# vibhaska/delta

Hardware: AMD Instinct MI355X
Metric: log actions replayed/sec + achieved HBM GB/s, 1/2/4/8 GPU, 10M-file table (higher is better)
Workload: dtype u8/int64; 1 GPU; config 3: 10M-file checkpoint + 30 JSON commits, 16000032 actions -> 10000000 live files, 30% remove/re-add churn, retention cutoff; actions=16000032, json_bytes=1775145997, checkpoint_bytes=859787616, parallelism=single GPU

## Files before the change

delta_amd/csrc/engine.hip:

```cpp
#include <hip/hip_runtime.h>
#include <rccl/rccl.h>
#include <dlfcn.h>
#include <sys/mman.h>
#include <unistd.h>
#include <sys/stat.h>
#include <fcntl.h>
#include <thread>

#include <algorithm>
#include <cmath>
#include <atomic>
#include <functional>
#include <type_traits>
#include <cstring>
#include <cctype>
#include <cerrno>
#include <cstdlib>
#include <cstdio>
#include <map>
#include <chrono>
#include <condition_variable>
#include <memory>
#include <mutex>
#include <string>
// ... 484 lines not shown
  std::vector<std::string> paths;
  std::vector<int> max_def, max_rep;
  std::vector<bool> present;
  std::vector<uint64_t> levels;
  std::vector<PageDesc> pages;
  DBuf<PageDesc> d_pages;
  uint32_t dict_entries = 0;
  DBuf<uint8_t> d_arena;
  std::vector<SnapPage> snap_pages;
  std::vector<uint32_t> chunk_base, block_page, chunk_page;
  std::vector<CopyJob> copy_jobs;
  uint32_t nchunks = 0;
  DBuf<SnapPage> d_snap;
  DBuf<uint32_t> d_chunk_base, d_block_page, d_chunk_page;
  DBuf<CopyJob> d_copy;
  DBuf<uint32_t> s_spec_exit, s_vis, s_entry, s_spec_first, s_assumed, s_region, s_chunk_out, s_chunk_out_start,
      s_chunk_elems, s_pages_bad, s_block_chunk, s_page_mark;
  DBuf<uint8_t> s_chunk_flag;
  DBuf<unsigned long long> s_region_count;
  std::vector<uint32_t> wg_chunk0;
  DBuf<uint32_t> d_wg_chunk0;
  uint64_t snap_in_bytes = 0, snap_out_bytes = 0, copy_bytes = 0;
  uint64_t snap_elements = 0;
  std::vector<InflatePage> gz_pages;
  DBuf<InflatePage> d_gz;
  uint64_t gz_in_bytes = 0, gz_out_bytes = 0;
  uint32_t ba_pages = 0;
  uint64_t ba_vals = 0;
  std::vector<uint2> ba_tiles;
  DBuf<uint2> d_ba_tiles;
  DBuf<uint32_t> s_ba_vals, s_ba_ok, s_ba_count, s_ba_tile_cnt;
  DBuf<uint64_t> s_ba_tile_off, s_ba_kept;
  DBuf<uint32_t> s_ba_link;
  std::vector<uint32_t> dl_pages;
  uint32_t dl_fc = 0, dl_groups = 0, dl_chunks = 0;
  uint64_t dl_tab = 0, dl_blk = 0;
  DBuf<uint32_t> d_dl_pages, s_dl_cnt;
  DBuf<uint64_t> s_dl_tab, s_dl_blk, s_dl_size, d_dl_out, d_dl_sized;
  DBuf<uint8_t> dl_arena;
  std::vector<uint64_t> dl_out, dl_sized_bytes;
  bool dl_sized = false;
  uint64_t dl_sizings = 0, dl_arena_bytes = 0;
};

struct HostBytes {
  uint8_t* p = nullptr;
  size_t n = 0, cap = 0;
  bool pinned = false;
  HostBytes() = default;
  HostBytes(const HostBytes&) = delete;
  HostBytes& operator=(const HostBytes&) = delete;
  ~HostBytes() { release(); }
  void release() {
    if (p) {
      if (pinned) (void)hipHostFree(p);
      else std::free(p);
    }
    p = nullptr;
    n = cap = 0;
  }
  void alloc(size_t bytes, size_t pad, bool pin) {
    release();
    cap = bytes + pad;
    pinned = pin;
    if (pin && hipHostMalloc(reinterpret_cast<void**>(&p), std::max<size_t>(cap, 1), hipHostMallocDefault) != hipSuccess) {
      (void)hipGetLastError();
// ... 492 lines not shown
    dbuf = DBuf<T>(s.ctx, vec.size());
    if (!vec.empty())
      HIP_OK(hipMemcpyAsync(dbuf.p, vec.data(), vec.size() * sizeof(T), hipMemcpyHostToDevice, s.ctx->stream));
  };
  up(P.d_snap, P.snap_pages);
  if (!P.gz_pages.empty()) up(P.d_gz, P.gz_pages);
  up(P.d_chunk_base, P.chunk_base);
  up(P.d_chunk_page, P.chunk_page);
  up(P.d_block_page, P.block_page);
  up(P.d_copy, P.copy_jobs);
  up(P.d_wg_chunk0, P.wg_chunk0);
  P.s_spec_exit = DBuf<uint32_t>(s.ctx, P.nchunks);
  P.s_vis = DBuf<uint32_t>(s.ctx, uint64_t(P.nchunks) * (snappy_chunk_bytes() / 32));
  P.s_entry = DBuf<uint32_t>(s.ctx, P.nchunks);
  P.s_spec_first = DBuf<uint32_t>(s.ctx, P.nchunks);
  P.s_assumed = DBuf<uint32_t>(s.ctx, P.nchunks);
  P.s_region = DBuf<uint32_t>(s.ctx, P.nchunks);
  P.s_block_chunk = DBuf<uint32_t>(s.ctx, P.block_page.size() + 1);
  P.s_chunk_flag = DBuf<uint8_t>(s.ctx, P.nchunks);
  P.s_region_count = DBuf<unsigned long long>(s.ctx, 1);
  P.s_chunk_out = DBuf<uint32_t>(s.ctx, P.nchunks);
  P.s_chunk_out_start = DBuf<uint32_t>(s.ctx, P.nchunks);
  P.s_chunk_elems = DBuf<uint32_t>(s.ctx, P.nchunks);
  P.s_pages_bad = DBuf<uint32_t>(s.ctx, P.snap_pages.size());
  P.s_page_mark = DBuf<uint32_t>(s.ctx, P.snap_pages.size());
  P.s_ba_vals = DBuf<uint32_t>(s.ctx, P.ba_vals);
  up(P.d_ba_tiles, P.ba_tiles);
  P.s_ba_tile_cnt = DBuf<uint32_t>(s.ctx, P.ba_tiles.size());
  P.s_ba_tile_off = DBuf<uint64_t>(s.ctx, P.ba_tiles.size() + 1);
  P.s_ba_kept = DBuf<uint64_t>(s.ctx, P.ba_tiles.size() * 256);
  P.s_ba_link = DBuf<uint32_t>(s.ctx, P.ba_tiles.size() * 3);
  P.s_ba_ok = DBuf<uint32_t>(s.ctx, P.ba_pages);
  P.s_ba_count = DBuf<uint32_t>(s.ctx, P.ba_pages);
  if (!P.dl_pages.empty()) {
    std::stable_partition(P.dl_pages.begin(), P.dl_pages.end(), [&](uint32_t i) { return P.pages[i].encoding == 7; });
    for (size_t k = 0; k < P.dl_pages.size(); ++k) {
      PageDesc& d = P.pages[P.dl_pages[k]];
      d.dl_slot = uint32_t(k);
      if (d.encoding == 7) {
        ++P.dl_fc;
        P.dl_groups = std::max(P.dl_groups, (d.num_values + 63) / 64);
      }
    }
    up(P.d_dl_pages, P.dl_pages);
    P.s_dl_tab = DBuf<uint64_t>(s.ctx, P.dl_tab);
    P.s_dl_blk = DBuf<uint64_t>(s.ctx, 2 * P.dl_blk);
    P.s_dl_cnt = DBuf<uint32_t>(s.ctx, P.dl_pages.size());
    P.s_dl_size = DBuf<uint64_t>(s.ctx, 2 * P.dl_pages.size());
    P.d_dl_out = DBuf<uint64_t>(s.ctx, P.dl_pages.size());
    P.d_dl_sized = DBuf<uint64_t>(s.ctx, P.dl_pages.size());
  }
  for (PageDesc& d : P.pages) {
    d.src = pqb + d.src;
    d.dst = arb + d.dst;
  }
  up(P.d_pages, P.pages);
}

static uint64_t scan_scratch_for(uint64_t n) {
  uint64_t b = scan_scratch_bytes(std::max<uint64_t>(n, uint64_t(1) << 23));
  if (const char* cap = std::getenv("DR_SCAN_SCRATCH_MAX")) b = std::min<uint64_t>(b, std::strtoull(cap, nullptr, 10));
  return b;
}
static ScanScratch ss(const DBuf<uint8_t>& b) { return ScanScratch{b.p, b.n}; }

static void pq_error(const PagePlan& P, uint32_t code, uint32_t gz, const std::string& what) {
// ... 1 lines not shown
    const uint32_t k = ~gz;
    const char* col = k < P.gz_pages.size() ? P.paths[size_t(P.pages[P.gz_pages[k].page].col)].c_str() : "?";
    fail(DR_E_PARQUET, fmt("corrupt gzip page in %s", col));
  }
  if (code != 0) fail(DR_E_PARQUET, fmt("%s failed (code %u)", what.c_str(), code));
}
static void pq_error(const PagePlan& P, const DBuf<uint32_t>& err, hipStream_t stream, const std::string& what) {
  const std::vector<uint32_t> w = d2h(err.p, 2, stream);
  pq_error(P, w[0], w[1], what);
}

static void decode_pages(dr_ctx* ctx, PagePlan& P, ParquetArgs& pa, DBuf<uint64_t>& dict_ptr, DBuf<uint32_t>& dict_len,
                         DBuf<uint32_t>& err, void*) {
  hipStream_t stream = ctx->stream;
  DBuf<uint8_t> own_scratch(ctx, scan_scratch_for(std::max<uint64_t>(P.nchunks, P.ba_tiles.size())));
  const ScanScratch scratch = ss(own_scratch);
  pa.pages = P.d_pages.p;
  pa.npages = uint32_t(P.pages.size());
  dict_ptr = DBuf<uint64_t>(ctx, P.dict_entries);
  dict_len = DBuf<uint32_t>(ctx, P.dict_entries);
  pa.dict_ptr = dict_ptr.p;
  pa.dict_len = dict_len.p;
  pa.error = err.p;
  pa.ba_vals = P.s_ba_vals.p;
  pa.ba_hit = nullptr;
  pa.ba_tiles = P.d_ba_tiles.p;
  pa.nba_tiles = uint32_t(P.ba_tiles.size());
  pa.ba_tile_cnt = P.s_ba_tile_cnt.p;
  pa.ba_tile_off = P.s_ba_tile_off.p;
  pa.ba_kept = P.s_ba_kept.p;
  pa.ba_link = P.s_ba_link.p;
  pa.ba_ok = P.s_ba_ok.p;
  pa.ba_count = P.s_ba_count.p;
  launch_page_copy(P.d_copy.p, uint32_t(P.copy_jobs.size()), stream);
  if (!P.snap_pages.empty()) {
    P.s_pages_bad.zero(stream);
    P.s_page_mark.zero(stream);
    P.s_chunk_flag.zero(stream);
    P.s_region_count.zero(stream);
    SnappyArgs sa{};
    sa.pages = P.d_snap.p;
    sa.npages = uint32_t(P.snap_pages.size());
    sa.chunk_base = P.d_chunk_base.p;
    sa.nchunks = P.nchunks;
    sa.spec_exit = P.s_spec_exit.p;
    sa.vis = P.s_vis.p;
    sa.entry = P.s_entry.p;
    sa.spec_first = P.s_spec_first.p;
    sa.assumed_exit = P.s_assumed.p;
    sa.chunk_flag = P.s_chunk_flag.p;
    sa.region = P.s_region.p;
    sa.region_count = P.s_region_count.p;
    sa.page_mark = P.s_page_mark.p;
    sa.chunk_out = P.s_chunk_out.p;
    sa.chunk_out_start = P.s_chunk_out_start.p;
    sa.chunk_elems = P.s_chunk_elems.p;
    sa.block_page = P.d_block_page.p;
    sa.block_chunk = P.s_block_chunk.p;
    sa.nblocks = uint32_t(P.block_page.size());
    sa.wg_chunk0 = P.d_wg_chunk0.p;
    sa.nwg = uint32_t(P.wg_chunk0.size());
    sa.pages_bad = P.s_pages_bad.p;
    sa.error = err.p;
    sa.chunk_page = P.d_chunk_page.p;
    DBuf<uint64_t> stamps, rstats;
    const bool dbg = std::getenv("DR_SNAP_DEBUG") != nullptr;
// ... 108 lines not shown
    pa.dl_tab = P.s_dl_tab.p;
    pa.dl_blk = P.s_dl_blk.p;
    pa.dl_cnt = P.s_dl_cnt.p;
    pa.dl_size = P.s_dl_size.p;
    launch_dl_scan(pa, stream);
    if (P.dl_fc) {
      if (!P.dl_sized) {
        const std::vector<uint64_t> sz = d2h(P.s_dl_size.p, 2 * uint64_t(ndl), stream);
        P.dl_out.assign(ndl, 0);
        P.dl_sized_bytes.assign(ndl, 0);
        uint64_t at = 0, longest = 0;
        for (uint32_t k = 0; k < P.dl_fc; ++k) {
          P.dl_out[k] = at;
          P.dl_sized_bytes[k] = sz[2 * k];
          at += (sz[2 * k] + 16 + 15) & ~uint64_t(15);
          longest = std::max(longest, sz[2 * k + 1]);
        }
        P.dl_arena = DBuf<uint8_t>(ctx, at + 64);
        P.dl_arena_bytes = at;
        P.dl_chunks = uint32_t((longest + 63) / 64);
        HIP_OK(hipMemcpyAsync(P.d_dl_out.p, P.dl_out.data(), ndl * sizeof(uint64_t), hipMemcpyHostToDevice, stream));
        HIP_OK(hipMemcpyAsync(P.d_dl_sized.p, P.dl_sized_bytes.data(), ndl * sizeof(uint64_t), hipMemcpyHostToDevice, stream));
        P.dl_sized = true;
        ++P.dl_sizings;
      }
      pa.dl_out = P.d_dl_out.p;
      pa.dl_sized = P.d_dl_sized.p;
      pa.dl_arena = P.dl_arena.p;
      launch_dl_expand(pa, P.dl_fc, P.dl_groups, P.dl_chunks, stream);
    }
  }
  launch_pq_dict(pa, stream);
  launch_pq_data(pa, stream);
}

static double now_s();

static void plan_checkpoint(StagedData& s) {
  const double t0 = now_s();
  uint64_t row_base = 0;
  for (CkPart& part : s.parts) {
    part.meta = pq::parse_footer(s.h_pq.data() + part.off, part.len);
    part.row_base = row_base;
    part.rows = 0;
    for (size_t gi = size_t(part.rg_lo); gi < part.rg_end(); ++gi) part.rows += uint64_t(part.meta.row_groups[gi].num_rows);
    row_base += part.rows;
  }
  s.ck_rows = row_base;
  if (s.parts.empty()) return;
  const pq::FileMeta& m0 = s.parts[0].meta;
  for (int c = 0; c < HC_N; ++c) {
    const pq::Leaf* l = m0.leaf(kHotPath[c]);
    s.has_col[c] = l != nullptr;
    if (l) {
      if (l->max_rep != 0) fail(DR_E_PARQUET, fmt("column %s is repeated", kHotPath[c]));
      s.max_def[c] = l->max_def;
      if (c == HC_ADD_PATH) s.add_def = l->def_of[0];
      if (c == HC_RM_PATH) s.rm_def = l->def_of[0];
    }
  }
  if (!s.has_col[HC_ADD_PATH]) fail(DR_E_PARQUET, "checkpoint has no add.path column");
  s.hot.paths.assign(kHotPath, kHotPath + HC_N);
  const double t1 = now_s();
  plan_pages(s, s.hot);
  const double t2 = now_s();
  for (CkPart& part : s.parts) decode_ck_nonfile(s, part, 0);
  if (std::getenv("DR_STAGE_DEBUG"))
    std::fprintf(stderr, "plan_checkpoint: %zu parts, footers %.3f s, pages %.3f s (%zu pages), non-file rows %.3f s\n",
                 s.parts.size(), t1 - t0, t2 - t1, s.hot.pages.size(), now_s() - t2);
}

struct StageSrc {
  int64_t version = 0;
  int32_t kind = DR_FILE_JSON, part = 0;
  const uint8_t* data = nullptr;
  uint64_t len = 0;
  std::string path;
  int32_t rg_lo = 0, rg_hi = -1;
};

static double now_s() {
  return std::chrono::duration<double>(std::chrono::steady_clock::now().time_since_epoch()).count();
}

static std::shared_ptr<StagedData> stage_sources(dr_ctx* ctx, std::vector<StageSrc>& src) {
  const bool dbg = std::getenv("DR_STAGE_DEBUG") != nullptr;
  const double t0 = now_s();
  auto s = std::make_shared<StagedData>();
  s->ctx = ctx;
  struct FdGuard {
    std::vector<int> fds;
    ~FdGuard() { for (int fd : fds) if (fd >= 0) close(fd); }
  } fdg;
  fdg.fds.assign(src.size(), -1);
  std::vector<uint8_t> ends_nl(src.size(), 0);
// ... 350 lines not shown
        HIP_OK(hipMemset(phase, 0, 16 * sizeof(unsigned long long)));
      }
      ja.phase = phase;
      if (++phase_calls % 200 == 0) {
        unsigned long long h[16];
        HIP_OK(hipMemcpy(h, phase, sizeof(h), hipMemcpyDeviceToHost));
        if (h[4])
          std::fprintf(stderr, "k_json_lines<true> clocks per wave: stage %.0f tape %.0f walk %.0f (rounds %.0f, first round %.0f; tape scan %.0f emit %.0f) (%llu waves)\n",
                       double(h[0]) / double(h[4]), double(h[1]) / double(h[4]), double(h[2]) / double(h[4]),
                       double(h[3]) / double(h[4]), double(h[5]) / double(h[4]), double(h[6]) / double(h[4]),
                       double(h[7]) / double(h[4]), h[4]);
        if (h[8] + h[9] + h[10] + h[11])
          std::fprintf(stderr, "k_apply_commit apply clocks: post-parse %.0f append %.0f touch %.0f delta %.0f\n",
                       double(h[8]) / double(h[4]), double(h[9]) / double(h[4]), double(h[10]) / double(h[4]),
                       double(h[11]) / double(h[4]));
        if (h[12] + h[13])
          std::fprintf(stderr, "k_apply_commit clocks: stage %.0f newlines %.0f walk %.0f apply %.0f expiry %.0f readback %.0f\n",
                       double(h[0]) / double(h[4]), double(h[1]) / double(h[4]), double(h[2]) / double(h[4]),
                       double(h[6]) / double(h[4]), double(h[12]) / double(h[4]), double(h[13]) / double(h[4]));
      }
    }
    if (defer_tail && fuse1 && tail_post) pp.parse_deferred = true;
    else launch_json_parse(ja, s2);
    if (!tail_post) launch_json_hard(ja, s2);
    if (overlap) {
      HIP_OK(hipEventCreateWithFlags(&ov.done, hipEventDisableTiming));
      HIP_OK(hipEventRecord(ov.done, s2));
    }
  }
  DBuf<uint8_t> cdefs;
  DBuf<int64_t> cival[HC_N];
  DBuf<uint64_t> csptr[HC_N];
  DBuf<uint32_t> cslen[HC_N];
  DBuf<uint64_t> dict_ptr;
  DBuf<uint32_t> dict_len, pq_err;
  if (R) {
    DR_STAGE("decode.checkpoint", stream);
    ParquetArgs pa{};
    pa.ncols = HC_N;
    cdefs = DBuf<uint8_t>(ctx, uint64_t(HC_N) * R);
    cdefs.zero(stream);
    for (int c = 0; c < HC_N; ++c) {
      if (c == HC_ADD_PATH || c == HC_RM_PATH) {
        csptr[c] = DBuf<uint64_t>(ctx, R);
        cslen[c] = DBuf<uint32_t>(ctx, R);
      } else {
        cival[c] = DBuf<int64_t>(ctx, R);
      }
      pa.cols[c] = FlatColumn{cdefs.p + uint64_t(c) * R, nullptr, cival[c].p, csptr[c].p, cslen[c].p};
    }
    pq_err = DBuf<uint32_t>(ctx, 2);
    pq_err.zero(stream);
    decode_pages(ctx, s.hot, pa, dict_ptr, dict_len, pq_err, scratch.p);
    CkptAssembleArgs ca{};
    ca.add_path = pa.cols[HC_ADD_PATH];
    ca.add_size = pa.cols[HC_ADD_SIZE];
    ca.rm_path = pa.cols[HC_RM_PATH];
    ca.rm_delts = pa.cols[HC_RM_DELTS];
    ca.add_def = s.add_def;
    ca.rm_def = s.rm_def;
    ca.add_path_max = s.max_def[HC_ADD_PATH];
    ca.add_size_max = s.has_col[HC_ADD_SIZE] ? s.max_def[HC_ADD_SIZE] : 255;
    ca.rm_path_max = s.max_def[HC_RM_PATH];
    ca.rm_delts_max = s.has_col[HC_RM_DELTS] ? s.max_def[HC_RM_DELTS] : 255;
    ca.has_rm = s.has_col[HC_RM_PATH] ? 1 : 0;
    ca.nrows = R;
    ca.row_base = 0;
    ca.act = act;
    ca.special_count = counters.p + 0;
    ca.special_bytes = counters.p + 1;
    launch_ckpt_assemble(ca, stream);
  }
  if (ov.done) {
    HIP_OK(hipStreamWaitEvent(stream, ov.done, 0));
  }
  if (R) HIP_OK(hipMemcpyAsync(counters.p + 7, pq_err.p, 2 * sizeof(uint32_t), hipMemcpyDeviceToDevice, stream));
  if (canonicalize) {
    DR_STAGE("canonicalize", stream);
    int64_t hint = s.canon_need.load();
    if (hint < 0 && ctx->opt.canon_hint >= 0) hint = ctx->opt.canon_hint;
    uint64_t cap = 0;
    if (hint < 0 && R == 0 && json_len <= (uint64_t(64) << 20)) {
// ... 4369 lines not shown
```

delta_amd/csrc/k_parquet.hip:

```cpp
#include "delta_enc.h"
#include "dev_common.h"
#include "kernels.h"

namespace dr {
namespace dev {

enum PqErr : uint32_t { PQE_SNAPPY = 1, PQE_LEVELS = 2, PQE_VALUES = 3, PQE_DICT = 4, PQE_ENCODING = 5 };

__device__ __forceinline__ void set_err(uint32_t* e, uint32_t code) { atomicCAS(e, 0u, code); }

__device__ __forceinline__ int level_width(int max_level) {
  int w = 0;
  while ((1 << w) <= max_level) ++w;
  return max_level == 0 ? 0 : w;
}

struct Rle {
  const uint8_t* p;
  const uint8_t* end;
  int width;
  uint32_t left;
  bool packed;
  uint32_t value;
  const uint8_t* pk;
// ... 212 lines not shown
  const uint64_t nx = p + 4 + w;
  if (nx > S || (w && !(in ? stage_u8(st, k + 4) : b[p + 4]))) return false;
  *next = nx;
  return true;
}
__device__ __forceinline__ uint64_t ba_kept_st(const uint8_t* b, uint64_t S, int64_t q0, const BaStage& st) {
  if (q0 + int64_t(BA_POS) <= 0 || q0 >= int64_t(S)) return 0ull;
  const uint4* a4 = reinterpret_cast<const uint4*>(st.w) + (q0 - st.t0) / 16;
  uint64_t z0 = 0;
  uint32_t z1 = 0;
#pragma unroll
  for (int v = 0; v < 5; ++v) {
    const uint4 x = a4[v];
    const uint32_t m = zero_nibble(x.x) | (zero_nibble(x.y) << 4) | (zero_nibble(x.z) << 8) | (zero_nibble(x.w) << 12);
    if (v < 4) z0 |= uint64_t(m) << (16 * v);
    else z1 = m;
  }
  auto zs = [&](int k) { return (z0 >> k) | (uint64_t(z1) << (64 - k)); };
  const uint64_t cm = zs(2) & zs(3) & (~zs(4) | (z0 & zs(1)));
  uint64_t kept = 0;
  for (uint64_t m = cm; m;) {
    const int j = __builtin_ctzll(m);
    m &= m - 1;
    const int64_t p = q0 + j;
    if (p < 0) continue;
    uint64_t nx, nn;
    if (ba_cand_st(b, S, uint64_t(p), &nx, st) && (nx == S || ba_cand_st(b, S, nx, &nn, st))) kept |= 1ull << j;
  }
  return kept;
}

__global__ void __launch_bounds__(BA_T) k_ba_count(ParquetArgs a) {
  __shared__ uint32_t red[BA_T / 64];
  __shared__ uint32_t tfirst[BA_T], tsucc[BA_T];
  __shared__ unsigned long long wbal[BA_T / 64];
  __shared__ uint32_t tile_bad;
  __shared__ __attribute__((aligned(16))) uint32_t stw[(BA_TILE + BA_MARGIN) / 4 + 8];
  const BaTile tl = ba_tile(a, blockIdx.x);
  BaStage st{stw, tl.q0 - int64_t(BA_POS) * int64_t(threadIdx.x), 0};
  if (tl.ok) {
    const int64_t hi = min(st.t0 + int64_t(BA_TILE + BA_MARGIN), int64_t(tl.S) + 16);
    const uint64_t nb = hi > st.t0 ? uint64_t(hi - st.t0) & ~uint64_t(15) : 0;
    const uint4* g4 = reinterpret_cast<const uint4*>(tl.b + st.t0);
    uint4* s4 = reinterpret_cast<uint4*>(stw);
    constexpr uint32_t PER = ((BA_TILE + BA_MARGIN) / 16 + BA_T - 1) / BA_T;
    const uint32_t nv = uint32_t(nb / 16);
    if (nv) {
      uint4 v[PER];
#pragma unroll
      for (uint32_t k = 0; k < PER; ++k) v[k] = gload16(g4 + min(threadIdx.x + k * BA_T, nv - 1));
#pragma unroll
      for (uint32_t k = 0; k < PER; ++k)
        if (threadIdx.x + k * BA_T < nv) s4[threadIdx.x + k * BA_T] = v[k];
    }
    st.n = nb;
  }
  if (threadIdx.x == 0) tile_bad = 0;
  __syncthreads();
  const uint64_t km = tl.ok ? (st.n >= uint64_t(tl.q0 - st.t0) + 80 ? ba_kept_st(tl.b, tl.S, tl.q0, st)
                                                                    : ba_kept(tl.b, tl.S, tl.q0))
                            : 0ull;
  a.ba_kept[uint64_t(blockIdx.x) * BA_T + threadIdx.x] = km;
  auto succ = [&](uint64_t p) -> uint64_t {
    const uint64_t k = p - uint64_t(st.t0);
    return p + 4 + (k + 8 <= st.n ? stage_u32(st, k) : load_u32(tl.b + p));
  };
  const uint32_t t = threadIdx.x, wv = t >> 6, ln = t & 63u;
// ... 10 lines not shown
      cbad |= nx != p;
      nx = succ(p);
    }
    cfirst = uint32_t(p0);
    clsucc = uint32_t(nx);
  }
  tfirst[t] = cfirst;
  tsucc[t] = clsucc;
  const unsigned long long bal = __ballot(km != 0ull);
  if (ln == 0) wbal[wv] = bal;
  __syncthreads();
  if (km) {
    uint32_t u = BA_NONE;
    const unsigned long long above = ln == 63 ? 0ull : (wbal[wv] >> (ln + 1)) << (ln + 1);
    if (above) {
      u = wv * 64 + uint32_t(__builtin_ctzll(above));
    } else {
      for (uint32_t x = wv + 1; x < BA_T / 64; ++x)
        if (wbal[x]) { u = x * 64 + uint32_t(__builtin_ctzll(wbal[x])); break; }
    }
    if (cbad || (u != BA_NONE && tfirst[u] != clsucc)) tile_bad = 1;
  }
  uint32_t* link = a.ba_link + 3ull * blockIdx.x;
  if (t == 0) {
    int lo = -1, hi = -1;
    for (uint32_t x = 0; x < BA_T / 64; ++x)
      if (wbal[x]) {
        if (lo < 0) lo = int(x * 64 + __builtin_ctzll(wbal[x]));
        hi = int(x * 64 + 63 - __builtin_clzll(wbal[x]));
      }
    link[0] = lo < 0 ? BA_NONE : tfirst[lo];
    link[1] = hi < 0 ? BA_NONE : tsucc[hi];
  }
  const uint32_t s = block_sum(uint32_t(__builtin_popcountll(km)), red);
  if (threadIdx.x == 0) {
    a.ba_tile_cnt[blockIdx.x] = s;
    if (a.ba_tiles[blockIdx.x].y == 0) a.ba_ok[tl.pg->ba_slot] = tl.ok ? 1u : 0u;
    link[2] = tile_bad;
  }
}

__global__ void __launch_bounds__(BA_T) k_ba_write(ParquetArgs a) {
  __shared__ uint32_t wsum[BA_T / 64];
  const BaTile tl = ba_tile(a, blockIdx.x);
  if (!tl.ok) return;
  const PageDesc pg = *tl.pg;
  uint64_t km = a.ba_kept[uint64_t(blockIdx.x) * BA_T + threadIdx.x];
  const uint32_t c = uint32_t(__builtin_popcountll(km));
  const int lane = threadIdx.x & 63, wv = threadIdx.x >> 6;
  uint32_t incl = c;
  for (int o = 1; o < 64; o <<= 1) {
    const uint32_t v = __shfl_up(incl, o, 64);
    if (lane >= o) incl += v;
  }
  if (lane == 63) wsum[wv] = incl;
  __syncthreads();
  uint32_t woff = 0;
  for (int k = 0; k < wv; ++k) woff += wsum[k];
  const uint32_t first = uint32_t(pg.hit_base);
  const uint64_t rank0 = a.ba_tile_off[blockIdx.x] - a.ba_tile_off[first] + woff + incl - c;
  const uint64_t cap = pg.usize / 4 + 2;
  const uint64_t boff = uint64_t(tl.b - reinterpret_cast<const uint8_t*>(pg.dst));
  uint32_t* vals = a.ba_vals + pg.ba_base;
  uint64_t o = rank0;
  while (km) {
    const int j = __builtin_ctzll(km);
    km &= km - 1;
    if (o < cap) vals[o] = uint32_t(uint64_t(tl.q0 + j) + boff);
    ++o;
  }
  const bool last = blockIdx.x + 1 == a.nba_tiles || a.ba_tiles[blockIdx.x + 1].x != a.ba_tiles[blockIdx.x].x;
// ... 405 lines not shown
  }
  const bool dict = pg.encoding == 2 || pg.encoding == 8;
  const bool rle_bool = pg.encoding == 3 && pg.phys == 0;
  Rle ir;
  ir.init(p, p, 0);
  if (dict) {
    if (pg.dict < 0) { if (tid == 0) set_err(a.error, PQE_DICT); return; }
    const int w = p < end ? *p : 0;
    ir.init(p + 1, end, w);
  } else if (rle_bool) {
    ir.init(p + 4, end, 1);
  } else if (pg.encoding != 0 && !DL) {
    if (tid == 0) set_err(a.error, PQE_ENCODING);
    return;
  }
  constexpr bool dl = DL;
  uint32_t dl_n = 0;
  const uint64_t* dl_tab = nullptr;
  const uint8_t* dl_bytes = nullptr;
  if constexpr (DL) {
    dl_n = a.dl_cnt[pg.dl_slot];
    if (dl_n == DL_BAD) return;
    dl_tab = a.dl_tab + pg.dl_base;
    dl_bytes = pg.encoding == 7 ? a.dl_arena + a.dl_out[pg.dl_slot] : reinterpret_cast<const uint8_t*>(pg.dst);
  }
  const uint32_t dict_base = dict ? a.pages[pg.dict].dict_base : 0;
  const uint32_t dict_n = dict ? a.pages[pg.dict].num_values : 0;
  const uint32_t width = pg.phys == 2 ? 8 : pg.phys == 1 ? 4 : 0;
  ByteArrayWalker wk;
  const bool ba_fast = pg.phys == 6 && !dict && pg.ba && a.ba_ok[pg.ba_slot];
  const uint32_t* ba_vals = a.ba_vals + pg.ba_base;
  const uint32_t ba_n = ba_fast ? a.ba_count[pg.ba_slot] : 0;
  const uint8_t* body = reinterpret_cast<const uint8_t*>(pg.dst);
  const bool walk = pg.phys == 6 && !dict && !ba_fast && !dl;
  if (walk && wv == 0) wk.init(p, end, lane);
  if (tid == 0) s_bad = 0;
  uint64_t vbase = 0;
  for (uint32_t s0 = 0; s0 < pg.num_values; s0 += SEG) {
    const uint32_t n = min(SEG, pg.num_values - s0);
    if (pg.max_rep > 0) {
      repr.expand(reps, n, tid, PQD_T);
      if (repr.bad) { if (tid == 0) set_err(a.error, PQE_LEVELS); return; }
    }
    if (pg.max_def > 0) {
      defr.expand(defs, n, tid, PQD_T);
      if (defr.bad) { if (tid == 0) set_err(a.error, PQE_LEVELS); return; }
    } else {
      for (uint32_t i = tid; i < n; i += PQD_T) defs[i] = 0;
    }
    __syncthreads();
    uint32_t nv = 0;
    for (uint32_t b = 0; b < n; b += PQD_T) {
      const uint32_t i = b + tid;
      const bool isv = i < n && int(defs[i]) == pg.max_def;
      const unsigned long long m = __ballot(isv);
      if (lane == 0) wcnt[wv] = uint32_t(__popcll(m));
      __syncthreads();
      uint32_t before = nv, tot = 0;
      for (int k = 0; k < PQD_T / 64; ++k) {
        before += k < wv ? wcnt[k] : 0u;
        tot += wcnt[k];
      }
      if (isv) idxs[i] = before + uint32_t(__popcll(m & ((1ull << lane) - 1ull)));
      nv += tot;
      __syncthreads();
    }
// ... 21 lines not shown
      if ((vbase + nv + 7) / 8 > uint64_t(end - p)) { if (tid == 0) set_err(a.error, PQE_VALUES); return; }
    } else {
      if (tid == 0) set_err(a.error, PQE_ENCODING);
      return;
    }
    __syncthreads();
    for (uint32_t i = tid; i < n; i += PQD_T) {
      const uint64_t row = pg.row_base + s0 + i;
      const uint8_t d = defs[i];
      col.def[row] = d;
      if (pg.max_rep > 0) col.rep[row] = reps[i];
      if (int(d) != pg.max_def) continue;
      const uint32_t k = idxs[i];
      if (dict) {
        const uint32_t j = vlen[k];
        if (j >= dict_n) { set_err(a.error, PQE_DICT); continue; }
        if (pg.phys == 6) {
          col.sptr[row] = a.dict_ptr[dict_base + j];
          col.slen[row] = a.dict_len[dict_base + j];
        } else {
          col.ival[row] = int64_t(a.dict_ptr[dict_base + j]);
        }
      } else if (rle_bool) {
        col.ival[row] = vlen[k] & 1;
      } else if (dl) {
        const uint64_t ent = dl_tab[vbase + k];
        if (pg.phys == 6) {
          col.sptr[row] = reinterpret_cast<uint64_t>(dl_bytes + (ent >> 32));
          col.slen[row] = uint32_t(ent);
        } else {
          col.ival[row] = int64_t(ent);
        }
      } else if (ba_fast) {
        const uint32_t off = ba_vals[vbase + k];
        col.sptr[row] = reinterpret_cast<uint64_t>(body + off + 4);
        col.slen[row] = load_u32(body + off);
      } else if (pg.phys == 6) {
        col.sptr[row] = vptr[k];
        col.slen[row] = vlen[k];
      } else if (width == 8) {
        col.ival[row] = int64_t(load_u64(p + 8 * (vbase + k)));
      } else if (width == 4) {
        col.ival[row] = int64_t(int32_t(load_u32(p + 4 * (vbase + k))));
      } else {
        const uint64_t b = vbase + k;
        col.ival[row] = (p[b >> 3] >> (b & 7)) & 1;
      }
    }
    vbase += nv;
    __syncthreads();
  }
  if (dl && vbase != dl_n && tid == 0) set_err(a.error, PQE_VALUES);
}

__global__ void __launch_bounds__(PQD_T) k_pq_data(ParquetArgs a) {
  if (blockIdx.x < a.npages) pq_data_body<false>(a, blockIdx.x);
}
__global__ void __launch_bounds__(PQD_T) k_pq_data_dl(ParquetArgs a) {
  if (blockIdx.x < a.ndl) pq_data_body<true>(a, a.dl_pages[blockIdx.x]);
}

constexpr uint32_t ASM_T = 256, ASM_STAGE = 8192;
__device__ __forceinline__ void asm_wave_sync() {
  __builtin_amdgcn_fence(__ATOMIC_RELEASE, "wavefront");
  __builtin_amdgcn_wave_barrier();
  __builtin_amdgcn_fence(__ATOMIC_ACQUIRE, "wavefront");
}
__global__ void __launch_bounds__(ASM_T) k_ckpt_assemble(CkptAssembleArgs a) {
  __shared__ __attribute__((aligned(16))) uint8_t stage[ASM_T / 64][ASM_STAGE + 32];
  const uint64_t r = uint64_t(blockIdx.x) * blockDim.x + threadIdx.x;
  const bool live = r < a.nrows;
  const uint64_t idx = a.row_base + r;
  uint8_t kind = K_NONE, flags = F_FROM_CKPT;
  const uint8_t* path = nullptr;
  uint32_t plen = 0;
  int64_t size = 0, delts = 0;
  const int ad = live ? int(a.add_path.def[r]) : 0;
  const int rd = live && a.has_rm ? int(a.rm_path.def[r]) : 0;
  if (live && ad >= a.add_def) {
    kind = K_ADD;
    if (ad == a.add_path_max) {
      path = reinterpret_cast<const uint8_t*>(a.add_path.sptr[r]);
      plen = a.add_path.slen[r];
    } else {
      flags |= F_PATH_NULL;
    }
    if (a.add_size.def[r] == a.add_size_max) size = a.add_size.ival[r];
  } else if (live && a.has_rm && rd >= a.rm_def) {
    kind = K_REMOVE;
    if (rd == a.rm_path_max) {
      path = reinterpret_cast<const uint8_t*>(a.rm_path.sptr[r]);
      plen = a.rm_path.slen[r];
    } else {
      flags |= F_PATH_NULL;
    }
    if (a.rm_delts.def && a.rm_delts.def[r] == a.rm_delts_max) {
      delts = a.rm_delts.ival[r];
      flags |= F_HAS_DELTS;
    }
  }
  const bool hashed = (kind == K_ADD || kind == K_REMOVE) && !(flags & F_PATH_NULL);
  uint64_t lo = hashed ? reinterpret_cast<uint64_t>(path) : ~0ull;
  uint64_t hi = hashed ? reinterpret_cast<uint64_t>(path) + plen : 0ull;
  for (int o = 32; o > 0; o >>= 1) {
    lo = min(lo, (uint64_t)__shfl_xor((unsigned long long)lo, o, 64));
    hi = max(hi, (uint64_t)__shfl_xor((unsigned long long)hi, o, 64));
  }
  const uint64_t a0 = lo & ~uint64_t(15);
  const bool staged = hi > lo && hi - a0 <= ASM_STAGE;
  uint8_t* stw = stage[threadIdx.x >> 6];
  if (staged) {
    const uint32_t nq = uint32_t((hi - a0 + 15) >> 4);
    const uint4* src = reinterpret_cast<const uint4*>(a0);
    for (uint32_t k = threadIdx.x & 63u; k < nq; k += 64) reinterpret_cast<uint4*>(stw)[k] = src[k];
    asm_wave_sync();
  }
  uint64_t key = 0;
  if (hashed) {
    const uint8_t* hp = staged ? stw + (reinterpret_cast<uint64_t>(path) - a0) : path;
    if (path_is_special(hp, plen)) {
      flags |= F_SPECIAL_PATH;
      atomicAdd(reinterpret_cast<unsigned long long*>(a.special_count), 1ull);
      atomicAdd(reinterpret_cast<unsigned long long*>(a.special_bytes), (unsigned long long)(plen + 8));
    } else {
      key = path_key(hp, plen);
    }
  }
  if (!live) return;
  a.act.kind[idx] = kind;
  a.act.flags[idx] = flags;
  a.act.key[idx] = key;
  a.act.path_ptr[idx] = reinterpret_cast<uint64_t>(path);
  a.act.path_len[idx] = plen;
  if (a.act.path_ref) a.act.path_ref[idx] = pack_ref(reinterpret_cast<uint64_t>(path), plen);
  a.act.size[idx] = size;
  a.act.delts[idx] = delts;
  a.act.src_off[idx] = r;
  a.act.src_len[idx] = 0;
}

}

uint32_t ba_tile_bytes() { return dev::BA_TILE; }
void launch_ba_bounds(const ParquetArgs& a, hipStream_t st, ScanScratch scan_scratch) {
  if (!a.nba_tiles) return;
  DR_LAUNCH(dev::k_ba_count, dim3(a.nba_tiles), dim3(dev::BA_T), 0, st, a);
  launch_scan_u32(a.ba_tile_cnt, a.ba_tile_off, a.nba_tiles, scan_scratch, st);
  DR_LAUNCH(dev::k_ba_write, dim3(a.nba_tiles), dim3(dev::BA_T), 0, st, a);
}
void launch_dl_scan(const ParquetArgs& a, hipStream_t st) {
  if (a.ndl) DR_LAUNCH(dev::k_dl_scan, dim3(a.ndl), dim3(dev::DL_T), 0, st, a);
}
void launch_dl_expand(const ParquetArgs& a, uint32_t nfc, uint32_t groups, uint32_t chunks, hipStream_t st) {
  if (!nfc || !groups || !chunks) return;
  const uint32_t y = chunks < 256u ? chunks : 256u;
  DR_LAUNCH(dev::k_dl_fc_last, dim3(nfc, y), dim3(64), 0, st, a);
  DR_LAUNCH(dev::k_dl_fc_fill, dim3(nfc * groups, y), dim3(64), 0, st, a, groups);
}
// ... 16 lines not shown
```

delta_amd/csrc/kernels.h:

```cpp
#pragma once
#include <hip/hip_runtime.h>
#include <hip/hip_ext.h>
#include <cstdint>
#include "filter_plan.h"

namespace dr {

typedef bool (*LaunchHook)(void* user, const char* kernel, hipEvent_t* start, hipEvent_t* stop);
void set_launch_hook(LaunchHook hook, void* user);
bool launch_events(const char* kernel, hipEvent_t* start, hipEvent_t* stop);
void launch_grid_check(const char* kernel, dim3 grid, dim3 block);
#define DR_LAUNCH(K, GRID, BLOCK, SHM, ST, ...)                                     \
  do {                                                                              \
    ::dr::launch_grid_check(#K, dim3(GRID), dim3(BLOCK));                           \
    hipEvent_t dr_e0_ = nullptr, dr_e1_ = nullptr;                                  \
    if (::dr::launch_events(#K, &dr_e0_, &dr_e1_))                                  \
      hipExtLaunchKernelGGL(K, GRID, BLOCK, SHM, ST, dr_e0_, dr_e1_, 0u, __VA_ARGS__); \
    else                                                                            \
      hipLaunchKernelGGL(K, GRID, BLOCK, SHM, ST, __VA_ARGS__);                     \
  } while (0)

struct ActionArrays {
  uint8_t* kind;
  uint8_t* flags;
// ... 61 lines not shown

struct PageDesc {
  uint64_t src;
  uint64_t dst;
  uint32_t csize, usize;
  uint32_t num_values;
  int32_t kind;
  int32_t encoding;
  int32_t codec;
  int32_t col;
  int32_t phys;
  int32_t max_def;
  int32_t max_rep;
  int32_t dict;
  uint64_t row_base;
  int32_t v2_def_len, v2_rep_len, v2_compressed;
  uint32_t dict_base;
  int32_t ba;
  uint32_t ba_slot;
  uint64_t ba_base;
  uint64_t hit_base;
  int32_t dl;
  uint32_t dl_slot;
  uint64_t dl_base;
  uint64_t dl_blk_base;
};

struct FlatColumn {
  uint8_t* def;
  uint8_t* rep;
  int64_t* ival;
  uint64_t* sptr;
  uint32_t* slen;
};

struct ParquetArgs {
  PageDesc* pages;
  uint32_t npages;
  FlatColumn cols[8];
  int32_t ncols;
  uint64_t* dict_ptr;
  uint32_t* dict_len;
  uint32_t* error;
  uint32_t* ba_vals;
  uint32_t* ba_hit;
  uint32_t* ba_ok;
  uint32_t* ba_count;
  const uint2* ba_tiles;
  uint32_t nba_tiles;
  uint32_t* ba_tile_cnt;
  uint64_t* ba_tile_off;
  uint64_t* ba_kept;
  uint32_t* ba_link;
  const uint32_t* dl_pages;
  uint32_t ndl;
  uint64_t* dl_tab;
  uint64_t* dl_blk;
  uint32_t* dl_cnt;
  uint64_t* dl_size;
  const uint64_t* dl_out;
  const uint64_t* dl_sized;
  uint8_t* dl_arena;
};
constexpr uint32_t DL_BAD = 0xFFFFFFFFu;
DR_HD inline uint64_t dl_blk_entries(uint32_t num_values) { return 2 * (uint64_t(num_values) / 128 + 2); }
void launch_dl_scan(const ParquetArgs& a, hipStream_t st);
void launch_dl_expand(const ParquetArgs& a, uint32_t nfc, uint32_t groups, uint32_t chunks, hipStream_t st);
uint32_t ba_tile_bytes();
void launch_ba_bounds(const ParquetArgs& a, hipStream_t st, ScanScratch scan_scratch);

struct SnapPage {
  uint64_t in, out;
  uint32_t n_in, n_out;
  uint32_t block_base;
};
struct CopyJob { uint64_t src, dst, n; };
struct SnappyArgs {
  const SnapPage* pages;
  uint32_t npages;
  const uint32_t* chunk_base;
  uint32_t nchunks;
  uint32_t* spec_exit;
  uint32_t* vis;
  uint32_t* entry;
  uint32_t* spec_first;
  uint32_t* assumed_exit;
// ... 624 lines not shown
```

Baseline: 1.883 billion actions/s.

## Hash checkpoint paths during byte-array boundary pass and reuse keys in action build

The byte-array boundary counting kernel now also computes path hash keys for each value while the tile is still staged in shared memory, storing up to a fixed cap per tile. The page decode propagates these precomputed keys and a keyed flag per row, and the action-building kernel skips re-reading and re-hashing path bytes for keyed rows. String lengths are now derived from neighbouring offsets rather than loaded from the page. This aims to avoid a second pass over path bytes in global memory, at the cost of extra per-tile key buffers, a prefix scan in the count kernel and more per-row metadata writes.

```diff
diff --git a/delta_amd/csrc/engine.hip b/delta_amd/csrc/engine.hip
--- a/delta_amd/csrc/engine.hip
+++ b/delta_amd/csrc/engine.hip
@@ -540,6 +540,9 @@
   DBuf<uint32_t> s_ba_vals, s_ba_ok, s_ba_count, s_ba_tile_cnt;
   DBuf<uint64_t> s_ba_tile_off, s_ba_kept;
   DBuf<uint32_t> s_ba_link;
+  bool want_keys = false;
+  DBuf<uint64_t> s_ba_keys;
+  DBuf<uint32_t> s_ba_keyed;
   std::vector<uint32_t> dl_pages;
   uint32_t dl_fc = 0, dl_groups = 0, dl_chunks = 0;
   uint64_t dl_tab = 0, dl_blk = 0;
@@ -1098,6 +1101,10 @@
   P.s_ba_link = DBuf<uint32_t>(s.ctx, P.ba_tiles.size() * 3);
   P.s_ba_ok = DBuf<uint32_t>(s.ctx, P.ba_pages);
   P.s_ba_count = DBuf<uint32_t>(s.ctx, P.ba_pages);
+  if (P.want_keys && !P.ba_tiles.empty()) {
+    P.s_ba_keys = DBuf<uint64_t>(s.ctx, P.ba_tiles.size() * BA_KEY_CAP);
+    P.s_ba_keyed = DBuf<uint32_t>(s.ctx, P.ba_tiles.size());
+  }
   if (!P.dl_pages.empty()) {
     std::stable_partition(P.dl_pages.begin(), P.dl_pages.end(), [&](uint32_t i) { return P.pages[i].encoding == 7; });
     for (size_t k = 0; k < P.dl_pages.size(); ++k) {
@@ -1165,6 +1172,16 @@
   pa.ba_link = P.s_ba_link.p;
   pa.ba_ok = P.s_ba_ok.p;
   pa.ba_count = P.s_ba_count.p;
+  bool keys = false;
+  FlatColumn asked[8];
+  for (int c = 0; c < pa.ncols; ++c) keys |= (asked[c] = pa.cols[c]).skey != nullptr;
+  const bool keys_asked = keys;
+  if (keys && !P.s_ba_keys.p) {
+    for (int c = 0; c < pa.ncols; ++c) pa.cols[c].skey = nullptr, pa.cols[c].skst = nullptr;
+    keys = false;
+  }
+  pa.ba_keys = keys ? P.s_ba_keys.p : nullptr;
+  pa.ba_keyed = keys ? P.s_ba_keyed.p : nullptr;
   launch_page_copy(P.d_copy.p, uint32_t(P.copy_jobs.size()), stream);
   if (!P.snap_pages.empty()) {
     P.s_pages_bad.zero(stream);
@@ -1339,6 +1356,20 @@
   }
   launch_pq_dict(pa, stream);
   launch_pq_data(pa, stream);
+  if (keys_asked && std::getenv("DR_BA_DEBUG")) {
+    uint64_t got = 0, all = 0;
+    for (int c = 0; c < pa.ncols; ++c) {
+      if (!asked[c].skey) continue;
+      const std::vector<uint8_t> df = d2h(asked[c].def, P.levels[size_t(c)], stream);
+      const std::vector<uint8_t> ks = d2h(asked[c].skst, P.levels[size_t(c)], stream);
+      for (size_t r = 0; r < df.size(); ++r) {
+        all += int(df[r]) == P.max_def[size_t(c)];
+        got += ks[r] != 0;
+      }
+    }
+    std::fprintf(stderr, "ba keys: %llu of %llu values keyed in the boundary pass\n", (unsigned long long)got,
+                 (unsigned long long)all);
+  }
 }
 
 static double now_s();
@@ -1368,6 +1399,7 @@
   }
   if (!s.has_col[HC_ADD_PATH]) fail(DR_E_PARQUET, "checkpoint has no add.path column");
   s.hot.paths.assign(kHotPath, kHotPath + HC_N);
+  s.hot.want_keys = true;
   const double t1 = now_s();
   plan_pages(s, s.hot);
   const double t2 = now_s();
@@ -1784,22 +1816,29 @@
   DBuf<int64_t> cival[HC_N];
   DBuf<uint64_t> csptr[HC_N];
   DBuf<uint32_t> cslen[HC_N];
+  DBuf<uint64_t> ckey[HC_N];
   DBuf<uint64_t> dict_ptr;
   DBuf<uint32_t> dict_len, pq_err;
   if (R) {
     DR_STAGE("decode.checkpoint", stream);
     ParquetArgs pa{};
     pa.ncols = HC_N;
-    cdefs = DBuf<uint8_t>(ctx, uint64_t(HC_N) * R);
+    cdefs = DBuf<uint8_t>(ctx, uint64_t(HC_N + 2) * R);
     cdefs.zero(stream);
+    int nkey = 0;
     for (int c = 0; c < HC_N; ++c) {
       if (c == HC_ADD_PATH || c == HC_RM_PATH) {
         csptr[c] = DBuf<uint64_t>(ctx, R);
         cslen[c] = DBuf<uint32_t>(ctx, R);
+        ckey[c] = DBuf<uint64_t>(ctx, R);
       } else {
         cival[c] = DBuf<int64_t>(ctx, R);
       }
-      pa.cols[c] = FlatColumn{cdefs.p + uint64_t(c) * R, nullptr, cival[c].p, csptr[c].p, cslen[c].p};
+      pa.cols[c] = FlatColumn{cdefs.p + uint64_t(c) * R, nullptr, cival[c].p, csptr[c].p, cslen[c].p, nullptr, nullptr};
+      if (ckey[c].p) {
+        pa.cols[c].skey = ckey[c].p;
+        pa.cols[c].skst = cdefs.p + uint64_t(HC_N + nkey++) * R;
+      }
     }
     pq_err = DBuf<uint32_t>(ctx, 2);
     pq_err.zero(stream);
diff --git a/delta_amd/csrc/k_parquet.hip b/delta_amd/csrc/k_parquet.hip
--- a/delta_amd/csrc/k_parquet.hip
+++ b/delta_amd/csrc/k_parquet.hip
@@ -268,7 +268,9 @@
 
 __global__ void __launch_bounds__(BA_T) k_ba_count(ParquetArgs a) {
   __shared__ uint32_t red[BA_T / 64];
-  __shared__ uint32_t tfirst[BA_T], tsucc[BA_T];
+  __shared__ uint32_t tfs[2 * BA_T];
+  uint32_t* const tfirst = tfs;
+  uint32_t* const tsucc = tfs + BA_T;
   __shared__ unsigned long long wbal[BA_T / 64];
   __shared__ uint32_t tile_bad;
   __shared__ __attribute__((aligned(16))) uint32_t stw[(BA_TILE + BA_MARGIN) / 4 + 8];
@@ -345,11 +347,50 @@
     link[0] = lo < 0 ? BA_NONE : tfirst[lo];
     link[1] = hi < 0 ? BA_NONE : tsucc[hi];
   }
-  const uint32_t s = block_sum(uint32_t(__builtin_popcountll(km)), red);
+  const uint32_t c = uint32_t(__builtin_popcountll(km));
+  uint32_t incl = c;
+  for (int o = 1; o < 64; o <<= 1) {
+    const uint32_t v = __shfl_up(incl, o, 64);
+    if (ln >= uint32_t(o)) incl += v;
+  }
+  if (ln == 63) red[wv] = incl;
+  __syncthreads();
+  uint32_t s = 0, woff = 0;
+  for (uint32_t k = 0; k < BA_T / 64; ++k) {
+    woff += k < wv ? red[k] : 0u;
+    s += red[k];
+  }
   if (threadIdx.x == 0) {
     a.ba_tile_cnt[blockIdx.x] = s;
     if (a.ba_tiles[blockIdx.x].y == 0) a.ba_ok[tl.pg->ba_slot] = tl.ok ? 1u : 0u;
     link[2] = tile_bad;
+  }
+  if (!a.ba_keys) return;
+  const bool want = tl.ok && tl.pg->kind != PG_DICT && a.cols[tl.pg->col].skey != nullptr;
+  const bool keyed = want && s <= BA_KEY_CAP;
+  if (threadIdx.x == 0) a.ba_keyed[blockIdx.x] = keyed ? 1u : 0u;
+  if (!keyed) return;
+  uint16_t* cand = reinterpret_cast<uint16_t*>(tfs);
+  static_assert(BA_KEY_CAP * sizeof(uint16_t) <= sizeof(tfs) && BA_TILE <= 65536, "candidate list");
+  {
+    uint32_t o = woff + incl - c;
+    for (uint64_t m = km; m; m &= m - 1) cand[o++] = uint16_t(BA_POS * t + uint32_t(__builtin_ctzll(m)));
+  }
+  __syncthreads();
+  uint64_t* keys = a.ba_keys + uint64_t(blockIdx.x) * BA_KEY_CAP;
+  const uint8_t* stb = reinterpret_cast<const uint8_t*>(stw);
+  for (uint32_t r = t; r < s; r += BA_T) {
+    const uint64_t k = cand[r];
+    const uint64_t p = uint64_t(st.t0 + int64_t(k));
+    const bool in = k + 8 <= st.n;
+    const uint32_t len = in ? stage_u32(st, k) : load_u32(tl.b + p);
+    if (in && k + 4 + len <= st.n) {
+      const uint8_t* v = stb + k + 4;
+      keys[r] = path_is_special(v, len) ? 0ull : path_key(v, len);
+    } else {
+      const uint8_t* v = tl.b + p + 4;
+      keys[r] = path_is_special(v, len) ? 0ull : path_key(v, len);
+    }
   }
 }
 
@@ -821,6 +862,8 @@
   const uint32_t* ba_vals = a.ba_vals + pg.ba_base;
   const uint32_t ba_n = ba_fast ? a.ba_count[pg.ba_slot] : 0;
   const uint8_t* body = reinterpret_cast<const uint8_t*>(pg.dst);
+  const uint64_t ba_boff = uint64_t(p - body), ba_lead = uint64_t(reinterpret_cast<uintptr_t>(p) & 15);
+  const uint64_t ba_rank0 = ba_fast && col.skey ? a.ba_tile_off[pg.hit_base] : 0;
   const bool walk = pg.phys == 6 && !dict && !ba_fast && !dl;
   if (walk && wv == 0) wk.init(p, end, lane);
   if (tid == 0) s_bad = 0;
@@ -908,9 +951,19 @@
           col.ival[row] = int64_t(ent);
         }
       } else if (ba_fast) {
-        const uint32_t off = ba_vals[vbase + k];
+        const uint64_t vk = vbase + k;
+        const uint32_t off = ba_vals[vk];
+        const uint32_t nxt = vk + 1 < ba_n ? ba_vals[vk + 1] : pg.usize;
         col.sptr[row] = reinterpret_cast<uint64_t>(body + off + 4);
-        col.slen[row] = load_u32(body + off);
+        col.slen[row] = nxt - off - 4;
+        if (col.skey) {
+          const uint64_t tile = pg.hit_base + (uint64_t(off) - ba_boff + ba_lead) / BA_TILE;
+          const uint64_t lr = vk - (a.ba_tile_off[tile] - ba_rank0);
+          if (a.ba_keyed[tile] && lr < BA_KEY_CAP) {
+            col.skey[row] = a.ba_keys[tile * BA_KEY_CAP + lr];
+            col.skst[row] = 1;
+          }
+        }
       } else if (pg.phys == 6) {
         col.sptr[row] = vptr[k];
         col.slen[row] = vlen[k];
@@ -951,6 +1004,8 @@
   const uint8_t* path = nullptr;
   uint32_t plen = 0;
   int64_t size = 0, delts = 0;
+  bool keyed = false;
+  uint64_t pre = 0;
   const int ad = live ? int(a.add_path.def[r]) : 0;
   const int rd = live && a.has_rm ? int(a.rm_path.def[r]) : 0;
   if (live && ad >= a.add_def) {
@@ -958,6 +1013,7 @@
     if (ad == a.add_path_max) {
       path = reinterpret_cast<const uint8_t*>(a.add_path.sptr[r]);
       plen = a.add_path.slen[r];
+      if (a.add_path.skst && a.add_path.skst[r]) keyed = true, pre = a.add_path.skey[r];
     } else {
       flags |= F_PATH_NULL;
     }
@@ -967,6 +1023,7 @@
     if (rd == a.rm_path_max) {
       path = reinterpret_cast<const uint8_t*>(a.rm_path.sptr[r]);
       plen = a.rm_path.slen[r];
+      if (a.rm_path.skst && a.rm_path.skst[r]) keyed = true, pre = a.rm_path.skey[r];
     } else {
       flags |= F_PATH_NULL;
     }
@@ -976,8 +1033,9 @@
     }
   }
   const bool hashed = (kind == K_ADD || kind == K_REMOVE) && !(flags & F_PATH_NULL);
-  uint64_t lo = hashed ? reinterpret_cast<uint64_t>(path) : ~0ull;
-  uint64_t hi = hashed ? reinterpret_cast<uint64_t>(path) + plen : 0ull;
+  const bool rehash = hashed && !keyed;
+  uint64_t lo = rehash ? reinterpret_cast<uint64_t>(path) : ~0ull;
+  uint64_t hi = rehash ? reinterpret_cast<uint64_t>(path) + plen : 0ull;
   for (int o = 32; o > 0; o >>= 1) {
     lo = min(lo, (uint64_t)__shfl_xor((unsigned long long)lo, o, 64));
     hi = max(hi, (uint64_t)__shfl_xor((unsigned long long)hi, o, 64));
@@ -994,12 +1052,12 @@
   uint64_t key = 0;
   if (hashed) {
     const uint8_t* hp = staged ? stw + (reinterpret_cast<uint64_t>(path) - a0) : path;
-    if (path_is_special(hp, plen)) {
+    if (keyed ? pre == 0 : path_is_special(hp, plen)) {
       flags |= F_SPECIAL_PATH;
       atomicAdd(reinterpret_cast<unsigned long long*>(a.special_count), 1ull);
       atomicAdd(reinterpret_cast<unsigned long long*>(a.special_bytes), (unsigned long long)(plen + 8));
     } else {
-      key = path_key(hp, plen);
+      key = keyed ? pre : path_key(hp, plen);
     }
   }
   if (!live) return;
diff --git a/delta_amd/csrc/kernels.h b/delta_amd/csrc/kernels.h
--- a/delta_amd/csrc/kernels.h
+++ b/delta_amd/csrc/kernels.h
@@ -117,7 +117,10 @@
   int64_t* ival;
   uint64_t* sptr;
   uint32_t* slen;
-};
+  uint64_t* skey;
+  uint8_t* skst;
+};
+constexpr uint32_t BA_KEY_CAP = 640;
 
 struct ParquetArgs {
   PageDesc* pages;
@@ -137,6 +140,8 @@
   uint64_t* ba_tile_off;
   uint64_t* ba_kept;
   uint32_t* ba_link;
+  uint64_t* ba_keys;
+  uint32_t* ba_keyed;
   const uint32_t* dl_pages;
   uint32_t ndl;
   uint64_t* dl_tab;
```

After: 1.895 billion actions/s (median of 3 runs). Within noise of the previous version (+0.7%).
